# autowarefoundation/autoware_vision_pilot

Hardware: AMD Instinct MI355X
Metric: frames/sec (SceneSeg+Scene3D 1280x720, one camera per GPU: preprocess + shared encoder + 2 decoder(s) + decode per frame); p50 per-frame latency beside it (higher is better)
Workload: dtype fp16x3 (hi+lo fp16 pairs on the fp16 MFMA pipe, fp32 accumulate; fp32-class: floats within 1e-3 of the fp32 oracle, 0 class flips outside that float tolerance -- tie flips only, counted per pass in profiles/r06_parity_sweep.tsv); 1 GPU; BASELINE.json metric configuration: SceneSeg+Scene3D on one 1280x720 camera per GPU, batch 1, shared EfficientNet-B0 encoder (vp_create_shared), fp16x3; precision=fp16x3, parity_mode=True, frames_in_flight_per_gpu=3, net_input=1x3x320x640, gather=False

## Files before the change

autoware_vision_pilot_amd/csrc/engine_upconv.cpp:

```cpp
#include "engine_internal.hpp"

namespace vp {

namespace {

inline void tap_of(int q, int tt, int* a, int* d) {
  const int hr = q + tt - 1;
  const int o = hr >= 0 ? hr / 2 : -1;
  *d = hr - 2 * o;
  *a = o + 1 - q;
}

inline void split_half_d(double v, double pre, half_t* hi, half_t* lo, int keep_bits) {
  const double x = v * pre;
  if (!(std::fabs(x) <= 65504.0)) throw RangeError("composed up-sampling weight " + std::to_string(v) + " is outside the fp16 range the matrix pipe carries: re-scale the checkpoint");
  const half_t h = (half_t)x;
  *hi = h;
  *lo = truncate_lo((half_t)(x - (double)h), keep_bits);
}

}

void Engine::compose_upconv(const float* wt, const float* bt, const float* ws, const float* bs, const float* w3, const float* b3, int cin, int cm, int cout,
                            int cs, UpconvComposed* out) {
// ... 77 lines not shown
    std::vector<ComposeGemmParams> gv(gs.begin() + 9, gs.end());
    d_gv = dupload(gv);
    VP_HIP_CHECK(launch_compose_gemm(d_gv, 9, cout, 1, stream_));
  }
  out->wx.resize(n_wx);
  std::vector<double> wsb(n_ws), vs(cs > 0 ? (size_t)9 * cout : 0);
  copy_d2h(out->wx.data(), d_wx, n_wx * sizeof(double));
  copy_d2h(wsb.data(), d_ws, n_ws * sizeof(double));
  if (cs > 0) copy_d2h(vs.data(), d_vs, vs.size() * sizeof(double));
  for (void* q : {(void*)d_w3r, (void*)d_wtr, (void*)d_br, (void*)d_bsr, (void*)d_wx, (void*)d_ws, (void*)d_vs, (void*)d_gx, (void*)d_gs, (void*)d_gv})
    if (q) dfree(q);
  out->ws.assign((size_t)9 * cout * cs, 0.0);
  std::vector<double> V((size_t)9 * cout);
  for (int t = 0; t < 9; ++t)
    for (int co = 0; co < cout; ++co) {
      const double* row = wsb.data() + ((size_t)t * cout + co) * (cs + 1);
      for (int c = 0; c < cs; ++c) out->ws[((size_t)t * cout + co) * cs + c] = row[c];
      V[(size_t)t * cout + co] = row[cs] + (cs > 0 ? vs[(size_t)t * cout + co] : 0.0);
    }
  out->bias.assign((size_t)9 * cout, 0.0);
  for (int rc = 0; rc < 3; ++rc)
    for (int cc = 0; cc < 3; ++cc)
      for (int co = 0; co < cout; ++co) {
        double b = (double)b3[co];
        for (int ty = (rc == 0 ? 1 : 0); ty <= (rc == 2 ? 1 : 2); ++ty)
          for (int tx = (cc == 0 ? 1 : 0); tx <= (cc == 2 ? 1 : 2); ++tx) b += V[(size_t)(ty * 3 + tx) * cout + co];
        out->bias[(size_t)(rc * 3 + cc) * cout + co] = b;
      }
}

bool Engine::upconv_wanted() const { return !fp8_storage() && !dev_option_is("VP_UPCONV", '0') && (split() || !dev_option_is("VP_UPCONV_F16", '0')); }

Act* Engine::add_upconv(const std::string& name, const Act* in, const Act* skip_in, const std::vector<float>& wt, const std::vector<float>& bt,
                        const std::vector<float>& ws, const std::vector<float>& bs, const std::vector<float>& w3, const std::vector<float>& b3, int cm,
                        int cout, int act, int shape, int nsplit, const std::string& out_name) {
  const bool x1 = !split();
  if (x1 && in->C % 64 != 0) throw std::invalid_argument("composed up-sampling stage in an fp16 engine: input channels a multiple of 64: " + name);
  const int cin = in->Creal, cin_pad = in->C, cs = skip_in ? skip_in->Creal : 0, cs_pad = skip_in ? skip_in->C : 0;
  if (wt.size() != (size_t)cin * cm * 4 || bt.size() != (size_t)cm) throw std::runtime_error("convT weight size mismatch: " + name);
  if (w3.size() != (size_t)cout * cm * 9 || b3.size() != (size_t)cout) throw std::runtime_error("conv weight size mismatch: " + name);
  if (skip_in && (ws.size() != (size_t)cm * cs || bs.size() != (size_t)cm)) throw std::runtime_error("skip conv weight size mismatch: " + name);
  if (skip_in && (skip_in->H != in->H * 2 || skip_in->W != in->W * 2)) throw std::runtime_error("skip tensor size mismatch: " + name);
  for (const std::vector<float>* v : {&wt, &w3, skip_in ? &ws : nullptr})
    if (v)
      for (float x : *v)
        if (!(std::fabs(x) <= 65504.0f))
          throw RangeError("weight " + std::to_string(x) + " is outside the fp16 range the matrix pipe carries (|w| <= 65504): re-scale the checkpoint");
  UpconvComposed cw;
  compose_upconv(wt.data(), bt.data(), skip_in ? ws.data() : nullptr, skip_in ? bs.data() : nullptr, w3.data(), b3.data(), cin, cm, cout, cs, &cw);

  const int ncols = round_up(cout, 32), coutw = round_up(ncols, 128);
  const int cin_v = x1 ? cin_pad / 2 : cin_pad, cs_v = x1 ? round_up(cs_pad, 64) / 2 : cs_pad, chm = x1 ? 2 : 1, chunk_w = x1 ? 64 : 32;
  const int S = upconv_steps(cin_v, cs_v), n_chunks = upconv_chunks(cin_v, cs_v);
  std::vector<half_t> hi((size_t)4 * S * coutw * 32, (half_t)0.0f), lo(hi.size(), (half_t)0.0f);
  std::vector<float> post((size_t)4 * coutw, 1.0f), bias((size_t)9 * coutw, 0.0f);
  for (int k = 0; k < 9; ++k)
    for (int co = 0; co < cout; ++co) bias[(size_t)k * coutw + co] = (float)cw.bias[(size_t)k * cout + co];
  parallel_rows(4 * cout, [&](int r_begin, int r_end) {
    for (int r = r_begin; r < r_end; ++r) {
      const int phase = r / cout, co = r - phase * cout, py = phase >> 1, px = phase & 1;
      double amax = 0.0;
      for (int k = 0; k < 4; ++k) {
        const double* row = cw.wx.data() + ((size_t)(phase * 4 + k) * cout + co) * cin;
        for (int ci = 0; ci < cin; ++ci) amax = std::max(amax, std::fabs(row[ci]));
      }
      for (int t = 0; t < 9 && cs > 0; ++t) {
        const double* row = cw.ws.data() + ((size_t)t * cout + co) * cs;
        for (int c = 0; c < cs; ++c) amax = std::max(amax, std::fabs(row[c]));
      }
      const int sexp = prescale_exp((float)amax);
      const double pre = std::ldexp(1.0, sexp);
      post[(size_t)phase * coutw + co] = std::ldexp(1.0f, -sexp);
      for (int c = 0; c < n_chunks; ++c) {
        const UpconvChunk d = upconv_chunk(c, py, px, cin_v, cs_v);
        const int creal = d.skip ? cs : cin;
        for (int k = 0; k < d.nt; ++k) {
          const int a = d.a0 + (d.nb == 2 ? (k >> 1) : k), b = d.b0 + (d.nb == 2 ? (k & 1) : 0);
          const double* row;
          if (d.skip) {
            const int ty = d.qy != py ? 2 * a : 1, tx = d.qx != px ? 2 * b : 1;
            row = cw.ws.data() + ((size_t)(ty * 3 + tx) * cout + co) * cs;
          } else {
            row = cw.wx.data() + ((size_t)(phase * 4 + a * 2 + b) * cout + co) * cin;
          }
          for (int i = 0; i < chunk_w && chm * d.ch0 + i < creal; ++i) {
            const size_t dst = upconv_pack_index(phase, d.step0 + k, co, i & 31, S, coutw);
            if (x1) {
              half_t h, l;
              split_half_d(row[chm * d.ch0 + i], pre, &h, &l, wlo_keep_);
              (i >> 5 ? lo : hi)[dst] = h;
            } else {
              split_half_d(row[d.ch0 + i], pre, &hi[dst], &lo[dst], wlo_keep_);
            }
          }
        }
      }
    }
  });
  Act* out = new_act(out_name.empty() ? name : out_name, cout, in->H * 2, in->W * 2);
  UpconvParams p{};
  p.in_hi = in->hi;
  p.in_lo = x1 ? nullptr : in->lo;
  p.sk_hi = skip_in ? skip_in->hi : nullptr;
  p.sk_lo = (skip_in && !x1) ? skip_in->lo : nullptr;
  p.H = in->H;
  p.W = in->W;
  p.Cin = cin_pad;
  p.Cs = cs_pad;
  p.w_hi = dupload(hi);
  p.w_lo = dupload(lo);
  wbytes_[1] += 2 * (hi.size() + lo.size());
  p.bias = dupload(bias);
  p.wscale = dupload(post);
  p.CoutW = coutw;
  p.Ncols = ncols;
  p.Cstore = out->C;
  p.out_hi = out->hi;
  p.out_lo = x1 ? nullptr : out->lo;
  p.act = (x1 && act == ACT_GELU) ? ACT_GELU_F16 : act;
  const long long t16 = (long long)((in->H + 15) / 16) * ((in->W + 15) / 16), t8 = (long long)((in->H + 7) / 8) * ((in->W + 15) / 16);
  const int n_co = coutw / 128;
  int sh = shape;
  {
    int ot = -1, on = 0;
    if (sh < 0 && plan_override(name, &ot, &on)) {
      sh = ot;
      if (on > 0 && nsplit <= 0) nsplit = on;
    }
  }
  if (sh < 0) {
    const double eff6 = (double)in->H * in->W / (double)(t16 * 256), eff7 = (double)in->H * in->W / (double)(t8 * 128);
    const char* e = dev_option("VP_UPCONV_SHAPE");
    sh = e ? std::atoi(e) : ((eff7 > 1.1 * eff6 || cin_pad <= 128) ? 7 : 6);
  }
  if (sh != 6 && sh != 7) throw std::invalid_argument("composed up-sampling stage: shape 6 (16x16 patches, 8 waves) or 7 (8x16 patches, 4 waves): " + name);
  const long long blocks = (sh == 6 ? t16 : t8) * 4 * n_co;
  int ns = nsplit;
  if (ns <= 0) {
    const long long slots = sh == 6 ? 256 : 512;
    ns = (int)std::max<long long>(1, slots / blocks);
    const double slice_mb = 4.0 * in->H * in->W * coutw * 4.0 / 1e6;
    while (ns > 1 && ns * slice_mb > 26.0) --ns;
    while (ns > 1 && S / ns < 12) --ns;
    if (const char* e = dev_option("VP_UPCONV_NSPLIT")) ns = std::max(1, std::atoi(e));
  }
  ns = std::max(1, std::min(ns, n_chunks));
  p.nsplit = ns;
  {
    const long long px = sh == 6 ? 256 : 128, runs = ((long long)in->H * in->W + px - 1) / px;
    const char* e = dev_option("VP_UPCONV_COMPACT");
    const bool want = e ? e[0] == '1' : runs < (sh == 6 ? t16 : t8);
    p.compact = (!x1 && want && upconv_compact_fits(in->H, in->W, sh)) ? 1 : 0;
  }
  p.partial = ns > 1 ? static_cast<float*>(dalloc((size_t)ns * 4 * in->H * in->W * coutw * sizeof(float), false)) : nullptr;
  if (!upconv_supported(p, sh)) throw std::invalid_argument("composed up-sampling stage: shape not covered: " + name);
  Op op;
  op.name = name;
  op.kernel = std::string(x1 ? "upconv_x1" : "upconv_x3") + (sh == 6 ? "w8<co128,px256" : "w4<co128,px128") + (x1 ? ",k64>" : ">") + (ns > 1 ? "+splitk" : "");
  if (ns > 1) op.launch = "nsplit=" + std::to_string(ns);
  const double M2 = 4.0 * in->H * in->W;
  op.flops = 2.0 * (M2 * cin * cm + M2 * cs * cm + M2 * 9.0 * cm * cout);
  op.flops_executed = 2.0 * M2 * cout * (4.0 * cin + 9.0 * cs);
  op.bytes = (x1 ? 2.0 : 4.0) * ((M2 / 4 * cin + M2 * cs + M2 * cout) + cout * (16.0 * cin + 9.0 * cs));
  op.run = [p, sh](hipStream_t st) { return launch_upconv(p, sh, st); };
  op.writes = {out};
  ops_.push_back(std::move(op));
  return out;
}

}
```

autoware_vision_pilot_amd/csrc/kernels.hpp:

```cpp
#pragma once
#include "common.hpp"

namespace vp {

const char* dev_option(const char* key);
bool dev_option_is(const char* key, char first);

struct PreprocessParams {
  const uint8_t* frame;
  int stride;
  const int* xtab;
  const int* ytab;
  int out_h, out_w;
  int src_c[3];
  float mean[3], stdv[3];
  float* out;
  int norm_form;
};

struct PilResampleParams {
  const uint8_t* frame;
  int stride;
  int in_h, in_w, out_h, out_w;
  const int* hb;
// ... 239 lines not shown
  const float* w2;
  const float* b2;
  int sq, Creal;
  int frames;
};

struct MbBackParams {
  ActView in;
  SeParams se;
  const unsigned long long* zsums;
  const float* w2q;
  const float* b2;
  int sqp;
  const float* w;
  const float* bias;
  const float* wscale;
  ActView res;
  ActView out;
};

struct LetterboxParams {
  const uint8_t* frame;
  int stride;
  const int* xtab;
  const int* ytab;
  int new_w, new_h, pad_x, pad_y;
  int out_h, out_w;
  float* out;
};

struct Detection {
  float x1, y1, x2, y2, confidence;
  int class_id;
};

enum DetectRule { kDetectPerClass = 0, kDetectAgnostic = 1 };
struct DetectParams {
  const float* raw;
  int num_attrs, num_boxes;
  float conf_thresh, iou_thresh;
  float scale;
  int pad_x, pad_y, orig_w, orig_h;
  float* boxes;
  int* cls;
  Detection* out;
  int out_cap;
  int* count;
};
constexpr int kDetectMaxBoxes = 16384;

struct LetterboxPasteParams {
  const float* src;
  int new_w, new_h, pad_x, pad_y;
  int out_h, out_w;
  float* out;
};

struct FcParams {
  const float* x;
  const float* w;
  const uint8_t* w8;
  const float* wscale8;
  const float* b;
  float* out;
  int N, K, act;
  unsigned act_rows;
  int rows_kernel;
  const float* partial;
  int nslab, Kstride;
  float inv_hw;
};

bool fc_rows_ok(const FcParams& p);

struct CtxConv1Params {
  const float* map;
  int H, W;
  const float* w;
  const float* b;
  ActView out;
  int act;
  int scaled;
  float out_mul;
};

struct CtxExpConv1Params {
  FcParams fc;
  CtxConv1Params cv;
  int tile;
  int glanes;
};
bool ctx_exp_conv1_ok(const CtxExpConv1Params& p);
hipError_t launch_ctx_exp_conv1(const CtxExpConv1Params& p, hipStream_t st);

struct FusionParams {
  ActView f[5];
  int creal[5];
  int shift[5];
  ActView out;
  int Creal_out;
  int octets;
};
bool fusion_octets_ok(const FusionParams& p);

hipError_t launch_conv_gemm(const ConvGemmParams& p, int tile, int bk, bool split, hipStream_t st);
int conv_tile_co(int tile);
int conv_tile_px(int tile);
hipError_t launch_conv3x3_halo(const ConvGemmParams& p, int tile, bool split, hipStream_t st);
bool conv3x3_x3_supported(const ConvGemmParams& p, int shape);
hipError_t launch_conv3x3_x3(const ConvGemmParams& p, int shape, hipStream_t st);
int halo_tile_co(int tile);
int halo_tile_px(int tile);
int halo_tile_th(int tile);
bool conv3x3_f8_supported(const ConvGemmParams& p);
hipError_t launch_conv3x3_f8(const ConvGemmParams& p, hipStream_t st);
hipError_t launch_fp8_quantize(const half_t* in, size_t n, float mul, uint8_t* out, hipStream_t st);

int conv3x3_map_geometry(int H, int W);
bool conv3x3_map_shape_ok(int H, int W, int cin_pad, int coutw);
size_t conv3x3_map_pack_index(int co, int ci, int t, int cin_pad);
size_t conv3x3_map_pack_index_k32(int co, int ci, int t, int cin_pad);
bool conv3x3_map_supported(const ConvGemmParams& p);
hipError_t launch_conv3x3_map(const ConvGemmParams& p, hipStream_t st);
bool conv3x3_map2_shape_ok(int H, int W, int cin_pad, int coutw);
bool conv3x3_map2_supported(const ConvGemmParams& p);
size_t conv3x3_map2_pack_index(int co, int ci, int t, int cin_pad);
hipError_t launch_conv3x3_map2(const ConvGemmParams& p, hipStream_t st);
bool head_conv_supported(const ConvGemmParams& p);
hipError_t launch_head_conv(const ConvGemmParams& p, const void* zeros, hipStream_t st);
bool gemm_dma_shape_ok(int M, int ncols, int cin_pad, int cin2_pad, int cstore);
size_t gemm_dma_pack_index(int n, int k, int kw);
bool gemm_dma_supported(const ConvGemmParams& p, bool split);
hipError_t launch_gemm_dma(const ConvGemmParams& p, hipStream_t st);
bool convt_rs_supported(const ConvGemmParams& p, bool split);
int convt_rs_shape_case(int H, int W, int cin_pad, int cin2_pad, int ncols, int cstore);
hipError_t launch_convt_rs(const ConvGemmParams& p, hipStream_t st);
struct UpconvParams {
  const half_t* in_hi;
  const half_t* in_lo;
  const half_t* sk_hi;
  const half_t* sk_lo;
  int H, W, Cin, Cs;
  const half_t* w_hi;
  const half_t* w_lo;
  const float* bias;
  const float* wscale;
  int CoutW, Ncols, Cstore;
  half_t* out_hi;
  half_t* out_lo;
  int act;
  int nsplit;
  float* partial;
  int compact;
};
bool upconv_supported(const UpconvParams& p, int shape);
bool upconv_compact_fits(int H, int W, int shape);
struct UpconvChunk {
  int skip, ch0, qy, qx, nt, nb, a0, b0, step0;
};
__host__ __device__ inline UpconvChunk upconv_chunk(int c, int py, int px, int cin_pad, int cs_pad) {
  const int kcx = cin_pad >> 5, kcs = cs_pad >> 5;
  UpconvChunk d;
  if (c < kcx || kcs == 0) {
    d.skip = 0; d.ch0 = c << 5; d.qy = 0; d.qx = 0; d.nt = 4; d.nb = 2; d.a0 = 0; d.b0 = 0; d.step0 = 4 * c;
    return d;
  }
  const int r = c - kcx, cls = r / kcs, cc = r - cls * kcs;
  d.skip = 1;
  d.ch0 = cc << 5;
  d.qy = cls < 2 ? 1 - py : py;
  d.qx = (cls & 1) ? px : 1 - px;
  const int na = d.qy != py ? 2 : 1;
  d.nb = d.qx != px ? 2 : 1;
  d.a0 = na == 2 ? 0 : 1 - py;
  d.b0 = d.nb == 2 ? 0 : 1 - px;
  d.nt = na * d.nb;
  const int cls_step0 = cls == 0 ? 0 : (cls == 1 ? 4 : (cls == 2 ? 6 : 8));
  d.step0 = 4 * kcx + cls_step0 * kcs + cc * d.nt;
  return d;
}
__host__ __device__ inline int upconv_chunks(int cin_pad, int cs_pad) { return (cin_pad >> 5) + 4 * (cs_pad >> 5); }
__host__ __device__ inline int upconv_steps(int cin_pad, int cs_pad) { return 4 * (cin_pad >> 5) + 9 * (cs_pad >> 5); }
inline size_t upconv_pack_index(int phase, int step, int co, int i, int steps, int coutw) {
  const int i_sw = ((((i & 31) >> 3) ^ ((co >> 2) & 3)) << 3) | (i & 7);
  return (((size_t)phase * steps + step) * coutw + co) * 32 + i_sw;
}
hipError_t launch_upconv(const UpconvParams& p, int shape, hipStream_t st);
struct ComposeGemmParams {
  const float* a[4];
  const float* b[4];
  int pairs, M, N, K;
  double* c;
};
hipError_t launch_compose_gemm(const ComposeGemmParams* groups_dev, int n_groups, int M, int N, hipStream_t st);
hipError_t launch_preprocess(const PreprocessParams& p, hipStream_t st);
hipError_t launch_pil_resample(const PilResampleParams& p, hipStream_t st);
hipError_t launch_stem(const StemParams& p, hipStream_t st);
hipError_t launch_dwconv(const DwParams& p, hipStream_t st);
bool mbconv_front_supported(const MbFrontParams& p);
hipError_t launch_mbconv_front(const MbFrontParams& p, hipStream_t st);
hipError_t launch_letterbox(const LetterboxParams& p, hipStream_t st);
hipError_t launch_detect_nms(const DetectParams& p, DetectRule rule, hipStream_t st);
inline hipError_t launch_detect_decode_nms(const DetectParams& p, hipStream_t st) { return launch_detect_nms(p, kDetectPerClass, st); }
hipError_t launch_letterbox_paste(const LetterboxPasteParams& p, hipStream_t st);
bool mbconv_back_supported(const MbBackParams& p);
hipError_t launch_mbconv_back(const MbBackParams& p, hipStream_t st);
hipError_t launch_pool_partial(const PoolParams& p, hipStream_t st);
hipError_t launch_zero_u64(unsigned long long* p, size_t n, hipStream_t st);
constexpr int kSeMaxReplicas = 64;
hipError_t launch_se_gate_scale(const SeParams& se, const ScaleWParams& sw, hipStream_t st);
hipError_t launch_fc(const FcParams& p, hipStream_t st);
hipError_t launch_ctx_conv1(const CtxConv1Params& p, hipStream_t st);
hipError_t launch_fusion(const FusionParams& p, hipStream_t st);
hipError_t launch_decode_mask(const float* logits, int C, int HW, int mode, uint8_t* out, hipStream_t st);
hipError_t launch_resize_nearest(const uint8_t* src, int sw, const int* ytab, const int* xtab, int oh, int ow, uint8_t* dst,
                                 hipStream_t st);
hipError_t launch_resize_bilinear_f32(const float* src, int sw, const int* yi, const float* yf, const int* xi, const float* xf,
                                      int oh, int ow, float* dst, hipStream_t st);
hipError_t launch_minmax_f32(const float* src, size_t n, unsigned* mm, hipStream_t st);
constexpr int VP_PROBE_BLOCKS = 64;
hipError_t launch_finite_probe(const float* src, size_t n, unsigned* flags, hipStream_t st);
hipError_t launch_depth_colorize(const float* src, size_t n, const unsigned* mm, const uint8_t* lut, uint8_t* dst, hipStream_t st);
hipError_t launch_viz_blend(const uint8_t* mask, int mw, const int* ytab, const int* xtab, const uint8_t* frame, int stride, int oh, int ow,
                            const uint8_t* lut, int frame_is_rgb, uint8_t* dst, hipStream_t st);
hipError_t launch_nchw_to_act(const float* src, int Creal, const ActView& a, hipStream_t st);
hipError_t launch_act_to_nchw(const ActView& a, int Creal, float* dst, hipStream_t st, float mul = 1.0f);
hipError_t launch_act_absmax(const half_t* hi, const half_t* lo, int c, int h, int w, int c_pitch, unsigned* result, hipStream_t st);
constexpr int VP_HIST_BINS = 40, VP_HIST_EXP_MIN = -24, VP_HIST_WORDS = VP_HIST_BINS + 2;
hipError_t launch_act_exp_hist(const half_t* hi, const half_t* lo, int c, int h, int w, int c_pitch, unsigned long long* result, hipStream_t st);

hipError_t launch_chan_copy(const ActView& src, int src_off, const ActView& dst, int dst_off, int nch, hipStream_t st);
hipError_t launch_maxpool5(const ActView& src, int src_off, const ActView& dst, int dst_off, int nch, hipStream_t st);
bool sppf_pool_ok(const ActView& src, const ActView& dst, int nch);
hipError_t launch_sppf_pool(const ActView& src, const ActView& dst, int nch, hipStream_t st);
struct AttnParams {
  ActView qkv;
  ActView out;
  ActView vout;
  int heads, dk, dv;
  float scale;
  int qblock;
};
bool attention_block_ok(const AttnParams& p);
hipError_t launch_attention(const AttnParams& p, hipStream_t st);
struct DwPlainParams {
  ActView in, out;
  ActView add;
  const float* w;
  const float* b;
  int act;
  int scaled;
  float in_mul, add_mul, out_mul;
};
hipError_t launch_dwconv_plain(const DwPlainParams& p, hipStream_t st);

struct Upsample2CatParams {
  ActView a, b, out;
  int a_off, a_nch, b_off, b_nch;
};
bool upsample2_cat_ok(const Upsample2CatParams& p);
hipError_t launch_upsample2_cat(const Upsample2CatParams& p, hipStream_t st);
struct DetectHeadLevel {
  ActView box;
  ActView cls;
  int first;
  float stride;
  float box_mul, cls_mul;
};
struct DetectHeadParams {
  DetectHeadLevel lv[3];
  int nc, total;
  float* out;
  int scaled;
};
hipError_t launch_detect_head_decode(const DetectHeadParams& p, hipStream_t st);

struct RowpairConvParams {
  ActView in;
  int cin;
  const float* w;
  const float* b;
  ActView out;
  int replicate;
  int scaled;
  float in_mul, out_mul;
};
bool rowpair_conv_ok(const RowpairConvParams& p);
hipError_t launch_rowpair_conv(const RowpairConvParams& p, hipStream_t st);
struct LaneRowsHeadParams {
  ActView features;
  int cin;
  const float* w;
  const float* hw;
  float* out;
  int scaled;
  float in_mul;
};
bool lane_rows_head_ok(const LaneRowsHeadParams& p);
hipError_t launch_lane_rows_head(const LaneRowsHeadParams& p, hipStream_t st);

struct MetricRecord {
  int kind;
  unsigned I[3], P[3], G[3];
  unsigned nonfinite, n, kept;
  float q_lo, q_hi, q, mae, mel;
};
// ... 197 lines not shown
```

autoware_vision_pilot_amd/csrc/kernels_upconv.hip:

```cpp
#include <algorithm>
#include <cstdlib>

#include "conv_epilogue.hpp"
#include "lds_dma.hpp"

namespace vp {

namespace {

struct PixPhase {
  int y0, x0, H, W, py, px;
  __device__ __forceinline__ int operator()(int q) const {
    int rowbit, c;
    lane_to_px16(q & 31, rowbit, c);
    const int y = y0 + 2 * (q >> 5) + rowbit, x = x0 + c;
    return (y < H && x < W) ? (2 * y + py) * (2 * W) + 2 * x + px : -1;
  }
};
struct PixRun {
  int kA, kE, W, py, px;
  __device__ __forceinline__ int operator()(int q) const {
    int rowbit, c;
    lane_to_px16(q & 31, rowbit, c);
    const int k = kA + (q >> 5) * 32 + 16 * rowbit + c;
    if (k >= kE) return -1;
    const int y = k / W, x = k - y * W;
    return (2 * y + py) * (2 * W) + 2 * x + px;
  }
};
constexpr int upconv_halo_bytes(int TH, bool CPT) { return (CPT && TH == 8) ? 192 * 80 : (TH + 2) * 18 * 80; }
constexpr int upconv_halo_capacity(int nth) { return 3 * nth / 4; }
__device__ __forceinline__ int bias_class(int m, int H2, int W2) {
  const int Y = m / W2, X = m - Y * W2;
  return (Y == 0 ? 0 : (Y == H2 - 1 ? 2 : 1)) * 3 + (X == 0 ? 0 : (X == W2 - 1 ? 2 : 1));
}

}

#define VP_WAIT_VMCNT_RT(N)                       \
  do {                                            \
    const int n_ = (N);                           \
    if (n_ >= 16) { VP_WAIT_VMCNT(16); }          \
    else if (n_ >= 14) { VP_WAIT_VMCNT(14); }     \
    else if (n_ >= 12) { VP_WAIT_VMCNT(12); }     \
    else if (n_ >= 10) { VP_WAIT_VMCNT(10); }     \
    else if (n_ >= 8) { VP_WAIT_VMCNT(8); }       \
    else if (n_ >= 6) { VP_WAIT_VMCNT(6); }       \
    else if (n_ >= 4) { VP_WAIT_VMCNT(4); }       \
    else if (n_ >= 2) { VP_WAIT_VMCNT(2); }       \
    else { VP_WAIT_VMCNT(0); }                    \
  } while (0)

template <int CO_TILE, int TH, int WCO, int WPX, bool HDB, int ACT, bool SPLITK, bool X1 = false, int ABL = 0, bool CPT = false>
__global__ __launch_bounds__(64 * WCO * WPX, 2) void upconv_x3_kernel(const UpconvParams p) {
  constexpr int NTH = 64 * WCO * WPX;
  constexpr int TW = 16, ROWB = 80, HWD = TW + 2, HPX = (TH + 2) * HWD, PX = TH * TW;
  constexpr int HALO_BYTES = upconv_halo_bytes(TH, CPT), WROW = 64, W_BYTES = CO_TILE * WROW;
  constexpr int HCHUNKS = HPX * 4, HP = (HCHUNKS + NTH - 1) / NTH;
  constexpr int MT = CO_TILE / WCO / 32, NT = PX / WPX / 32;
  constexpr int NHB = HDB ? 2 : 1;
  constexpr int PL = 2;
  constexpr int HSTRIDE = HALO_BYTES;
  static_assert(MT >= 1 && NT >= 1 && HP <= 3, "tile shape");
  extern __shared__ __attribute__((aligned(16))) char smem[];
  char* const halo_base = smem;
  char* const w_base = smem + NHB * PL * HSTRIDE;

  const int tid = threadIdx.x, lane = tid & 63, wave = tid >> 6;
  const int wco = wave / WPX, wpx = wave % WPX;
  const int tiles_x = (p.W + TW - 1) / TW;
  const int n_px_tiles = CPT ? (p.H * p.W + PX - 1) / PX : tiles_x * ((p.H + TH - 1) / TH);
  const int n_co_tiles = p.CoutW / CO_TILE;
  int vid;
  {
    const int nwg = gridDim.x, q = nwg >> 3, r = nwg & 7, xcd = blockIdx.x & 7;
    vid = (xcd < r ? xcd * (q + 1) : r * (q + 1) + (xcd - r) * q) + (blockIdx.x >> 3);
  }
  int tile_px, tile_co, phase, zsplit = 0;
  if constexpr (SPLITK) {
    tile_px = vid % n_px_tiles;
    int rest = vid / n_px_tiles;
    tile_co = rest % n_co_tiles;
    rest /= n_co_tiles;
    phase = rest & 3;
    zsplit = rest >> 2;
  } else {
    tile_co = vid % n_co_tiles;
    const int rest = vid / n_co_tiles;
    phase = rest & 3;
    tile_px = rest >> 2;
  }
  const int py = phase >> 1, px = phase & 1;
  const int tyi = tile_px / tiles_x, txi = tile_px - tyi * tiles_x;
  const int y0 = tyi * TH, x0 = txi * TW;
  const int kA = tile_px * PX, kE = min(kA + PX, p.H * p.W);
  const int yA = kA / p.W, xA = kA - yA * p.W, yE = (kE - 1) / p.W, xE = (kE - 1) - yE * p.W;
  const int hrp = CPT ? p.W * ROWB + 256 : HWD * ROWB;
  const int tpy = CPT ? 0 : py, tpx = CPT ? 0 : px;
  const int co0 = tile_co * CO_TILE;
  const int CinV = X1 ? p.Cin >> 1 : p.Cin, CsV = X1 ? ((p.Cs + 63) >> 6) << 5 : p.Cs;
  constexpr int CHM = X1 ? 2 : 1;
  const half_t* const in_p1 = X1 ? p.in_hi + 32 : p.in_lo;
  const half_t* const sk_p1 = X1 ? p.sk_hi + 32 : p.sk_lo;
#define VP_SK_DEAD1(D) (X1 && (D).skip && CHM * (D).ch0 + 32 >= p.Cs)
  const int n_chunks = upconv_chunks(CinV, CsV);
  int cA = 0, cB = n_chunks;
  if constexpr (SPLITK) {
    cA = (int)(((long long)n_chunks * zsplit) / p.nsplit);
    cB = (int)(((long long)n_chunks * (zsplit + 1)) / p.nsplit);
  }

  const int h_lds0 = (tid >> 2) * ROWB + (tid & 3) * 16;
  constexpr int NW = NTH / 64, WPIECES = W_BYTES / 1024 / NW;
  static_assert(W_BYTES % (1024 * NW) == 0, "weight tile splits into 1 KiB pieces per wave");
  const size_t w_step = (size_t)p.CoutW * 32;
  typedef unsigned int u32x4 __attribute__((ext_vector_type(4)));
  const u32x4 zero4 = {0u, 0u, 0u, 0u};
  int b_ofs0;
  int b_ofs[NT];
  int nlj = NT;
  {
    int rowbit, c;
    lane_to_px16(lane & 31, rowbit, c);
    b_ofs0 = ((2 * (wpx * NT) + rowbit) * HWD + c) * ROWB + (lane >> 5) * 16;
    if constexpr (CPT) {
#pragma unroll
      for (int j = 0; j < NT; ++j) {
        int k = kA + (wpx * NT + j) * 32 + 16 * rowbit + c;
        if (k >= kE) k = kA;
        const int y = k / p.W, x = k - y * p.W;
        b_ofs[j] = (y - yA) * hrp + (x - xA) * ROWB + (lane >> 5) * 16;
      }
      nlj = __builtin_amdgcn_readfirstlane(min(NT, max(0, (kE - kA + 31) / 32 - wpx * NT)));
    }
  }
  const int a_swz = ((lane & 31) >> 2) & 3;
  const int a_ofs0 = (wco * 32 + (lane & 31)) * WROW + (((lane >> 5) ^ a_swz) << 4);

  int h_gx[HP], h_gs[HP], h_ls[HP];
#pragma unroll
  for (int pc = 0; pc < HP; ++pc) {
    const int hidx = tid + NTH * pc;
    const int hp = hidx >> 2, ch = hidx & 3;
    int gy, gx;
    bool ok;
    if constexpr (CPT) {
      const int gw = p.W + 2, lg = py * gw + xA + px + hp, cnt = (yE - yA + 1) * gw + xE - xA + 2;
      const int r = lg / gw, cc = lg - r * gw;
      gy = yA - 1 + r;
      gx = cc - 1;
      ok = hp < cnt && (unsigned)gy < (unsigned)p.H && (unsigned)gx < (unsigned)p.W;
      h_ls[pc] = hp < cnt ? (r - py) * hrp + (cc - xA - px) * ROWB + ch * 16 : -1;
    } else {
      const int hy = hp / HWD, hx = hp - hy * HWD;
      gy = y0 - 1 + hy;
      gx = x0 - 1 + hx;
      ok = hidx < HCHUNKS && (unsigned)gy < (unsigned)p.H && (unsigned)gx < (unsigned)p.W && hy >= py && hy <= py + TH && hx >= px && hx <= px + TW;
    }
    h_gx[pc] = ok ? (gy * p.W + gx) * p.Cin + ch * 8 : -1;
    h_gs[pc] = ok ? (4 * gy * p.W + 2 * gx) * p.Cs + ch * 8 : -1;
  }
  const UpconvChunk dA = upconv_chunk(cA, py, px, CinV, CsV);
  const int S = (cB < n_chunks ? upconv_chunk(cB, py, px, CinV, CsV).step0 : upconv_steps(CinV, CsV)) - dA.step0;
  const size_t w_goff0 = ((size_t)phase * upconv_steps(CinV, CsV) + dA.step0) * w_step + co0 * 32 + wave * 512 + lane * 8;

  f32x16_t acc[MT][NT];
#pragma unroll
  for (int i = 0; i < MT; ++i)
#pragma unroll
    for (int j = 0; j < NT; ++j)
#pragma unroll
      for (int r = 0; r < 16; ++r) acc[i][j][r] = 0.0f;

  h8_t fa[2][MT], fal[2][MT], fb[2][NT], fbl[2][NT];
  u32x4 rh_hi[HP], rh_lo[HP];
#pragma unroll
  for (int r = 0; r < HP; ++r) rh_hi[r] = rh_lo[r] = zero4;

#define VP_DMA_W(WOFS, SIDX)                                                                 \
  if (!(ABL & 128) || (SIDX) < 2) {                                                          \
    const size_t base_ = (size_t)(SIDX) * w_step + w_goff0;                                  \
    char* dst_ = w_base + (WOFS) + wave * 1024;                                              \
    _Pragma("unroll") for (int pc = 0; pc < WPIECES; ++pc) {                                 \
      VP_GLOBAL_LOAD_LDS16(p.w_hi + base_ + pc * NW * 512, dst_ + pc * NW * 1024);           \
      VP_GLOBAL_LOAD_LDS16(p.w_lo + base_ + pc * NW * 512, dst_ + W_BYTES + pc * NW * 1024); \
    }                                                                                        \
  }
#define VP_LOAD_H(D)                                                                         \
  if (!(ABL & 1) || abl_prologue) {                                                          \
    const half_t* sh_ = (D).skip ? p.sk_hi : p.in_hi;                                        \
    const half_t* sl_ = (D).skip ? (VP_SK_DEAD1(D) ? p.sk_hi : sk_p1) : in_p1;               \
    const int add_ = (D).skip ? ((D).qy * 2 * p.W + (D).qx) * p.Cs + CHM * (D).ch0 : CHM * (D).ch0; \
    _Pragma("unroll") for (int pc = 0; pc < HP; ++pc) {                                      \
      const int g_ = (D).skip ? h_gs[pc] : h_gx[pc];                                         \
      const int o_ = (g_ >= 0 ? g_ + add_ : 0);                                              \
      rh_hi[pc] = *reinterpret_cast<const u32x4*>(sh_ + o_);                                 \
      rh_lo[pc] = *reinterpret_cast<const u32x4*>(sl_ + o_);                                 \
    }                                                                                        \
  }
#define VP_STORE_H(BUF, DEAD1)                                                               \
  if (!(ABL & 1) || abl_prologue)                                                            \
  _Pragma("unroll") for (int pc = 0; pc < HP; ++pc) {                                        \
    if (CPT ? h_ls[pc] >= 0 : tid + NTH * pc < HCHUNKS) {                                    \
      char* dst_ = halo_base + (BUF) * PL * HSTRIDE + (CPT ? h_ls[pc] : h_lds0 + pc * (NTH / 4) * ROWB); \
      *reinterpret_cast<u32x4*>(dst_) = h_gx[pc] >= 0 ? rh_hi[pc] : zero4;                   \
      *reinterpret_cast<u32x4*>(dst_ + HSTRIDE) = (h_gx[pc] >= 0 && !(DEAD1)) ? rh_lo[pc] : zero4; \
    }                                                                                        \
  }
#define VP_READ_FRAGS(SET, WPTR, HPTR, TAPOFS)                                               \
  {                                                                                          \
    const char* wsrc_ = (WPTR) + (a_ofs0 ^ ((SET) * 32));                                    \
    if (!CPT || nlj > 0)                                                                     \
    _Pragma("unroll") for (int i = 0; i < MT; ++i) {                                         \
      fa[SET][i] = *reinterpret_cast<const h8_t*>(wsrc_ + i * WCO * 32 * WROW);              \
      fal[SET][i] = *reinterpret_cast<const h8_t*>(wsrc_ + W_BYTES + i * WCO * 32 * WROW);   \
    }                                                                                        \
    if constexpr (CPT) {                                                                     \
      const char* hsrc_ = (HPTR) + (TAPOFS) + (SET) * 32;                                    \
      _Pragma("unroll") for (int j = 0; j < NT; ++j) {                                       \
        if (j >= nlj) continue;                                                              \
        fb[SET][j] = *reinterpret_cast<const h8_t*>(hsrc_ + b_ofs[j]);                       \
        fbl[SET][j] = *reinterpret_cast<const h8_t*>(hsrc_ + HSTRIDE + b_ofs[j]);            \
      }                                                                                      \
    } else {                                                                                 \
      const char* hsrc_ = (HPTR) + b_ofs0 + (TAPOFS) + (SET) * 32;                           \
      _Pragma("unroll") for (int j = 0; j < NT; ++j) {                                       \
        fb[SET][j] = *reinterpret_cast<const h8_t*>(hsrc_ + j * 2 * HWD * ROWB);             \
        fbl[SET][j] = *reinterpret_cast<const h8_t*>(hsrc_ + HSTRIDE + j * 2 * HWD * ROWB);  \
      }                                                                                      \
    }                                                                                        \
  }
#define VP_MFMA_RANGE(SET, Q0, Q1)                                                           \
  _Pragma("unroll") for (int q_ = (Q0); q_ < (Q1); ++q_) {                                   \
    const int i = q_ / NT, j = q_ % NT;                                                      \
    if constexpr (CPT) { if (j >= nlj) continue; }        \
    if constexpr ((ABL & 2) != 0) { acc[i][j][0] += (float)fa[SET][i][0] + (float)fal[SET][i][1] + (float)fb[SET][j][2] + (float)fbl[SET][j][3]; continue; } \
    if constexpr (X1) {                      \
      acc[i][j] = __builtin_amdgcn_mfma_f32_32x32x16_f16(fa[SET][i], fb[SET][j], acc[i][j], 0, 0, 0);   \
      acc[i][j] = __builtin_amdgcn_mfma_f32_32x32x16_f16(fal[SET][i], fbl[SET][j], acc[i][j], 0, 0, 0); \
      continue;                                                                              \
    }                                                                                        \
    acc[i][j] = __builtin_amdgcn_mfma_f32_32x32x16_f16(fal[SET][i], fb[SET][j], acc[i][j], 0, 0, 0); \
    acc[i][j] = __builtin_amdgcn_mfma_f32_32x32x16_f16(fa[SET][i], fbl[SET][j], acc[i][j], 0, 0, 0); \
    acc[i][j] = __builtin_amdgcn_mfma_f32_32x32x16_f16(fa[SET][i], fb[SET][j], acc[i][j], 0, 0, 0);  \
  }
#define VP_TAP_OFS(D, K) ((tpy + (D).a0 + ((D).nb == 2 ? ((K) >> 1) : (K))) * hrp + (tpx + (D).b0 + ((D).nb == 2 ? ((K) & 1) : 0)) * ROWB)

  bool abl_prologue = true;
  VP_LOAD_H(dA)
  VP_STORE_H(0, VP_SK_DEAD1(dA))
  VP_DMA_W(0, 0)
  if (S > 1) VP_DMA_W(PL * W_BYTES, 1)
  VP_WAIT_VMCNT(0);
  __syncthreads();
  UpconvChunk d = dA;
  UpconvChunk dn = dA;
  if (cA + 1 < cB) {
    dn = upconv_chunk(cA + 1, py, px, CinV, CsV);
    VP_LOAD_H(dn)
  }
  VP_READ_FRAGS(0, w_base, halo_base, VP_TAP_OFS(d, 0))
  abl_prologue = false;

  int c = cA, t = 0, s = 0, hb = 0;
  int w_cur = 0, w_nxt = PL * W_BYTES, w_fre = 2 * PL * W_BYTES;
#define VP_STEP(KIND, PREVLD)                                                                \
  {                                                                                          \
    const int tap_cur_ = VP_TAP_OFS(d, t);                                                   \
    const int tap_nxt_ = (KIND) == 0 ? VP_TAP_OFS(d, t + 1) : ((KIND) == 3 ? tap_cur_ : VP_TAP_OFS(dn, 0)); \
    const char* hbuf = halo_base + (HDB ? hb : 0) * PL * HSTRIDE;                            \
    const char* hbuf_next = (HDB && (KIND) != 0) ? halo_base + (hb ^ 1) * PL * HSTRIDE : hbuf; \
     \
     \
     \
    if constexpr (HDB && ((KIND) == 1 || (KIND) == 2)) { VP_STORE_H(hb ^ 1, VP_SK_DEAD1(dn)) }   \
     \
    if (s + 2 < S) VP_DMA_W(w_fre, s + 2)                                                    \
    __builtin_amdgcn_sched_barrier(0);                                                       \
    VP_MFMA_RANGE(0, 0, MT * NT / 2)                                                         \
    __builtin_amdgcn_sched_barrier(0);                                                       \
    VP_READ_FRAGS(1, w_base + w_cur, hbuf, tap_cur_)                                         \
    __builtin_amdgcn_sched_barrier(0);   \
    UpconvChunk dnn = dn;                                                                    \
    if constexpr (HDB && (KIND) == 1) {                                                      \
      dnn = upconv_chunk(c + 2, py, px, CinV, CsV);                                        \
      VP_LOAD_H(dnn)                                                                         \
    }                                                                                        \
    VP_MFMA_RANGE(0, MT * NT / 2, MT * NT)                                                   \
    __builtin_amdgcn_sched_barrier(0);                                                       \
     \
     \
    {                                                                                        \
      const int dma_n = s + 2 < S ? PL * WPIECES : 0;                                        \
      const int ld_prev = ((PREVLD) && t == 0) ? PL * HP : 0;                                \
      const int ld_this = (HDB && (KIND) == 1) ? PL * HP : 0;                                \
      VP_WAIT_VMCNT_RT(dma_n + ld_prev + ld_this);                                           \
    }                                                                                        \
     \
    VP_LDS_BARRIER();                                                                        \
    if constexpr (!HDB && ((KIND) == 1 || (KIND) == 2)) {                                    \
       \
       \
      VP_STORE_H(0, VP_SK_DEAD1(dn))                                                         \
      VP_LDS_BARRIER();                                                                      \
      if constexpr ((KIND) == 1) {                                                           \
        dnn = upconv_chunk(c + 2, py, px, CinV, CsV);                                      \
        VP_LOAD_H(dnn)                                                                       \
      }                                                                                      \
    }                                                                                        \
           \
    VP_READ_FRAGS(0, w_base + w_nxt, hbuf_next, tap_nxt_)                                    \
    __builtin_amdgcn_sched_barrier(0);                                                       \
    VP_MFMA_RANGE(1, 0, MT * NT)                                                             \
    __builtin_amdgcn_sched_barrier(0);                                                       \
                                    \
    {                                                                                        \
      const int w_old = w_cur;                                                               \
      w_cur = w_nxt;                                                                         \
      w_nxt = w_fre;                                                                         \
      w_fre = w_old;                                                                         \
    }                                                                                        \
    ++s;                                                                                     \
    if constexpr ((KIND) == 0) {                                                             \
      ++t;                                                                                   \
    } else {                                                                                 \
      ++c;                                                                                   \
      t = 0;                                                                                 \
      d = dn;                                                                                \
      dn = dnn;                                                                              \
      hb ^= 1;                                                                               \
    }                                                                                        \
  }
  while (c + 2 < cB) {
    while (t + 1 < d.nt) VP_STEP(0, true)
    VP_STEP(1, true)
  }
  if (c + 1 < cB) {
    while (t + 1 < d.nt) VP_STEP(0, true)
    VP_STEP(2, true)
  }
  while (t + 1 < d.nt) VP_STEP(0, false)
  VP_STEP(3, false)
#undef VP_STEP
#undef VP_SK_DEAD1
#undef VP_TAP_OFS
#undef VP_MFMA_RANGE
#undef VP_READ_FRAGS
#undef VP_STORE_H
#undef VP_LOAD_H
#undef VP_DMA_W

  const auto pix = [&] {
    if constexpr (CPT) return PixRun{kA, kE, p.W, py, px};
    else return PixPhase{y0, x0, p.H, p.W, py, px};
  }();
  if constexpr ((ABL & 16) != 0) {
    if (p.H == -12345) {
#pragma unroll
      for (int i = 0; i < MT; ++i)
#pragma unroll
        for (int j = 0; j < NT; ++j)
#pragma unroll
          for (int r = 0; r < 16; ++r) p.partial[(i * NT + j) * 16 + r + tid * 64] = acc[i][j][r];
    }
    return;
  }
  if constexpr (SPLITK) {
    const int M2 = 4 * p.H * p.W;
#pragma unroll
    for (int j = 0; j < NT; ++j) {
      const int m = pix((wpx * NT + j) * 32 + (lane & 31));
      if (m < 0) continue;
      float* row = p.partial + ((size_t)zsplit * M2 + m) * p.CoutW + co0 + 4 * (lane >> 5);
#pragma unroll
      for (int i = 0; i < MT; ++i)
#pragma unroll
        for (int g = 0; g < 4; ++g) {
          const f32x4_t v = {acc[i][j][4 * g + 0], acc[i][j][4 * g + 1], acc[i][j][4 * g + 2], acc[i][j][4 * g + 3]};
          *reinterpret_cast<f32x4_t*>(row + (i * WCO + wco) * 32 + 8 * g) = v;
        }
    }
    return;
  } else {
    constexpr int PITCH = CO_TILE * 2 + 16, STAGE_PLANE = PX * PITCH;
    static_assert(PL * STAGE_PLANE <= NHB * PL * HSTRIDE + 3 * PL * W_BYTES, "stage fits the main buffers");
    const float* const wsc = p.wscale + (size_t)phase * p.CoutW + co0;
    f32x4_t bb[NT][MT][4], sc[MT][4];
    int qpix[NT];
#pragma unroll
    for (int j = 0; j < NT; ++j) {
      qpix[j] = (wpx * NT + j) * 32 + (lane & 31);
      const int m = pix(qpix[j]);
      const float* const bsrc = p.bias + (size_t)(m >= 0 ? bias_class(m, 2 * p.H, 2 * p.W) : 4) * p.CoutW + co0;
#pragma unroll
      for (int i = 0; i < MT; ++i)
#pragma unroll
        for (int g = 0; g < 4; ++g) bb[j][i][g] = *reinterpret_cast<const f32x4_t*>(bsrc + (i * WCO + wco) * 32 + 4 * (lane >> 5) + 8 * g);
    }
#pragma unroll
    for (int i = 0; i < MT; ++i)
#pragma unroll
      for (int g = 0; g < 4; ++g) sc[i][g] = *reinterpret_cast<const f32x4_t*>(wsc + (i * WCO + wco) * 32 + 4 * (lane >> 5) + 8 * g);
    __syncthreads();
#pragma unroll
    for (int j = 0; j < NT; ++j) {
#pragma unroll
      for (int i = 0; i < MT; ++i) {
        const int cl = (i * WCO + wco) * 32 + 4 * (lane >> 5);
        char* row = smem + qpix[j] * PITCH + cl * 2;
#pragma unroll
        for (int g = 0; g < 4; ++g) {
          h4_t h, l;
#pragma unroll
          for (int r = 0; r < 4; ++r) {
            const float x = apply_act(fmaf(acc[i][j][4 * g + r], sc[i][g][r], bb[j][i][g][r]), ACT);
            h[r] = (half_t)x;
            if constexpr (!X1) l[r] = (half_t)(x - (float)h[r]);
          }
          *reinterpret_cast<h4_t*>(row + g * 16) = h;
          if constexpr (!X1) *reinterpret_cast<h4_t*>(row + STAGE_PLANE + g * 16) = l;
        }
      }
    }
    __syncthreads();
    constexpr int CPR = CO_TILE / 8, RPI = NTH / CPR;
    static_assert(NTH % CPR == 0 && PX % RPI == 0, "row loop shape");
    const int c8 = tid % CPR, r0 = tid / CPR;
    const int co = co0 + c8 * 8;
    if (co >= p.Ncols) return;
#pragma unroll 4
    for (int r = r0; r < PX; r += RPI) {
      const int m = pix(r);
      if (m < 0) continue;
      if constexpr ((ABL & 32) != 0) { if (p.H != -12345) continue; }
      const size_t o = (size_t)m * p.Cstore + co;
      *reinterpret_cast<h8_t*>(p.out_hi + o) = *reinterpret_cast<const h8_t*>(smem + r * PITCH + c8 * 16);
      if constexpr (!X1) *reinterpret_cast<h8_t*>(p.out_lo + o) = *reinterpret_cast<const h8_t*>(smem + STAGE_PLANE + r * PITCH + c8 * 16);
    }
  }
}

__global__ __launch_bounds__(256) void upconv_finish_kernel(const UpconvParams p) {
  const int H2 = 2 * p.H, W2 = 2 * p.W, M2 = H2 * W2;
  const int groups = p.Ncols >> 3;
  const long long t = (long long)blockIdx.x * 256 + threadIdx.x;
  if (t >= (long long)M2 * groups) return;
  const int m = (int)(t / groups), co = (int)(t % groups) * 8;
  float v[8] = {0.f, 0.f, 0.f, 0.f, 0.f, 0.f, 0.f, 0.f};
  for (int z = 0; z < p.nsplit; ++z) {
    const float* src = p.partial + ((size_t)z * M2 + m) * p.CoutW + co;
    const f32x4_t q0 = *reinterpret_cast<const f32x4_t*>(src), q1 = *reinterpret_cast<const f32x4_t*>(src + 4);
#pragma unroll
    for (int r = 0; r < 4; ++r) {
      v[r] += q0[r];
      v[4 + r] += q1[r];
    }
  }
  const int Y = m / W2, X = m - Y * W2;
  const int phase = (Y & 1) * 2 + (X & 1);
  const float* b = p.bias + (size_t)bias_class(m, H2, W2) * p.CoutW + co;
  const float* s = p.wscale + (size_t)phase * p.CoutW + co;
  h8_t hi, lo;
#pragma unroll
  for (int r = 0; r < 8; ++r) {
    const float x = apply_act(fmaf(v[r], s[r], b[r]), p.act);
    hi[r] = (half_t)x;
    lo[r] = (half_t)(x - (float)hi[r]);
  }
  const size_t o = (size_t)m * p.Cstore + co;
  *reinterpret_cast<h8_t*>(p.out_hi + o) = hi;
  if (p.out_lo) *reinterpret_cast<h8_t*>(p.out_lo + o) = lo;
}

bool upconv_compact_fits(int H, int W, int shape) {
  if ((shape != 6 && shape != 7) || H < 1 || W < 1 || (long long)H * W >= (1 << 24)) return false;
  const int PX = shape == 6 ? 256 : 128, nth = shape == 6 ? 512 : 256, th = shape == 6 ? 16 : 8;
  for (int kA = 0; kA < H * W; kA += PX) {
    const int kE = std::min(kA + PX, H * W), yA = kA / W, xA = kA - yA * W, yE = (kE - 1) / W, xE = (kE - 1) - yE * W;
    const long long cnt = (long long)(yE - yA + 1) * (W + 2) + xE - xA + 2;
    const long long bytes = (long long)(yE - yA + 1) * (W * 80 + 256) + (xE - xA + 1) * 80 + 80;
    if (cnt > upconv_halo_capacity(nth) || bytes > upconv_halo_bytes(th, true)) return false;
  }
  return true;
}

bool upconv_supported(const UpconvParams& p, int shape) {
  if (shape != 6 && shape != 7) return false;
  if (p.compact && (p.in_lo == nullptr || !upconv_compact_fits(p.H, p.W, shape))) return false;
  const bool x1 = p.in_lo == nullptr;
  if (!(p.in_hi && p.w_hi && p.w_lo && p.bias && p.wscale && p.out_hi && (x1 ? p.out_lo == nullptr : p.out_lo != nullptr))) return false;
  if (p.H < 1 || p.W < 1 || p.Cin < (x1 ? 64 : 32) || p.Cin % (x1 ? 64 : 32) != 0 || p.Cs % 32 != 0 || p.Cs < 0) return false;
  if (p.Cs > 0 && !(p.sk_hi && (x1 ? p.sk_lo == nullptr : p.sk_lo != nullptr))) return false;
  if (p.CoutW % 128 != 0 || p.Ncols % 8 != 0 || p.Ncols > p.CoutW || p.Cstore < p.Ncols) return false;
  if (!(p.act == (x1 ? ACT_GELU_F16 : ACT_GELU) || p.act == ACT_NONE)) return false;
  if (p.nsplit < 1 || p.nsplit > (x1 ? upconv_chunks(p.Cin >> 1, ((p.Cs + 63) >> 6) << 5) : upconv_chunks(p.Cin, p.Cs))) return false;
// ... 96 lines not shown
```

autoware_vision_pilot_amd/csrc/options.cpp:

```cpp
#include <atomic>
#include <cstring>
#include <deque>
#include <map>
#include <mutex>
#include <string>

#include "../../include/vp_hip.h"
#include "kernels.hpp"

namespace vp {
namespace {
std::mutex g_mu;
std::atomic<int> g_count{0};
std::map<std::string, const char*> g_opts;
std::deque<std::string> g_arena;
bool g_version_stale = true;
std::deque<std::string> g_versions;

const char* const kKeys[] = {"VP_MBCONV_FUSE", "VP_MBCONV_BACK", "VP_PROJ_SPLIT", "VP_FUSE_DECODE", "VP_AUTOTUNE", "VP_HEAD_CONV", "VP_CONVT_RS",
                             "VP_CONV3X3", "VP_HEAD_TILE5", "VP_X3_TILE", "VP_X3_MIN_WGS", "VP_MAP3X3", "VP_NSPLIT_PCT", "VP_NSPLIT_FORCE", "VP_X3_C64",
                             "VP_GEMM_DMA", "VP_GEMM_DMA_NSPLIT", "VP_CONVT_TILE", "VP_CONVT_BK", "VP_FUSE_SKIP", "VP_CONVT_RS_GROUPS", "VP_F16_BIG",
                             "VP_CTX3", "VP_MAP_TAPSPLIT", "VP_ATTN_BLOCK", "VP_F16_MAP", "VP_MAP_NSPLIT_PCT", "VP_MAP2", "VP_MAP2_SLOTS", "VP_X3_T16", "VP_MAP2_CAP_MB", "VP_MAP2_MIN_REGIONS", "VP_CTX_FUSE", "VP_MAP_MAX_M", "VP_F16_MIN_WGS", "VP_CONVT_RS_GROUPS_K288", "VP_PLAN_TARGET", "VP_UPCONV", "VP_UPCONV_SHAPE", "VP_UPCONV_NSPLIT", "VP_PLAN_OVERRIDE", "VP_WLO_KEEP_BITS", "VP_UPCONV_F16", "VP_UPCONV_COMPACT"};
}

const char* dev_option(const char* key) {
  if (g_count.load(std::memory_order_acquire) == 0) return nullptr;
  std::lock_guard<std::mutex> lk(g_mu);
  auto it = g_opts.find(key);
  return it == g_opts.end() ? nullptr : it->second;
}
bool dev_option_is(const char* key, char first) {
  const char* v = dev_option(key);
  return v != nullptr && v[0] == first;
}

}

extern "C" {

int vp_set_option(const char* key, const char* value) {
  if (!key) return VP_ERR_ARG;
  bool known = false;
  for (const char* k : vp::kKeys) known = known || std::strcmp(k, key) == 0;
  if (!known) return VP_ERR_ARG;
  if (value && std::strcmp(key, "VP_PLAN_TARGET") == 0 && std::strcmp(value, "latency") != 0 && std::strcmp(value, "throughput") != 0) return VP_ERR_ARG;
  std::lock_guard<std::mutex> lk(vp::g_mu);
  if (!value) {
    vp::g_opts.erase(key);
  } else {
    vp::g_arena.emplace_back(value);
    vp::g_opts[key] = vp::g_arena.back().c_str();
  }
  vp::g_version_stale = true;
  vp::g_count.store((int)vp::g_opts.size(), std::memory_order_release);
  return VP_OK;
}

const char* vp_get_option(const char* key) { return key ? vp::dev_option(key) : nullptr; }

void vp_clear_options(void) {
  std::lock_guard<std::mutex> lk(vp::g_mu);
  vp::g_opts.clear();
  vp::g_version_stale = true;
  vp::g_count.store(0, std::memory_order_release);
}

const char* vp_version(void) {
  std::lock_guard<std::mutex> lk(vp::g_mu);
  if (vp::g_version_stale) {
    std::string s = "libvp_hip 0.5 (gfx950; options:";
    if (vp::g_opts.empty()) s += " none";
    for (const auto& kv : vp::g_opts) s += std::string(" ") + kv.first + "=" + kv.second;
    s += ")";
    if (vp::g_versions.empty() || vp::g_versions.back() != s) vp::g_versions.push_back(s);
    vp::g_version_stale = false;
  }
  return vp::g_versions.back().c_str();
}

}
```

Baseline: 561.0 frames/s.

## Add statically unrolled tap schedule for up-conv input-channel chunks

Adds a specialised main loop for the composed up-sampling kernel that unrolls the four taps of each input-channel chunk with compile-time step kinds. This lets vmcnt waits use immediate counts instead of a runtime ladder, and interleaves weight DMA, halo loads and MFMA halves at fixed positions. The wave index used for LDS DMA addressing is also made wave-uniform through readfirstlane. The path is on by default for non-x1 kernels and can be disabled with an option. It adds code size and register pressure, and the hand-computed wait counts risk a correctness or hazard error if they are miscounted.

```diff
diff --git a/autoware_vision_pilot_amd/csrc/engine_upconv.cpp b/autoware_vision_pilot_amd/csrc/engine_upconv.cpp
--- a/autoware_vision_pilot_amd/csrc/engine_upconv.cpp
+++ b/autoware_vision_pilot_amd/csrc/engine_upconv.cpp
@@ -253,6 +253,7 @@
     const bool want = e ? e[0] == '1' : runs < (sh == 6 ? t16 : t8);
     p.compact = (!x1 && want && upconv_compact_fits(in->H, in->W, sh)) ? 1 : 0;
   }
+  p.xstatic = dev_option_is("VP_UPCONV_STATIC", '0') ? 0 : 1;
   p.partial = ns > 1 ? static_cast<float*>(dalloc((size_t)ns * 4 * in->H * in->W * coutw * sizeof(float), false)) : nullptr;
   if (!upconv_supported(p, sh)) throw std::invalid_argument("composed up-sampling stage: shape not covered: " + name);
   Op op;
diff --git a/autoware_vision_pilot_amd/csrc/kernels.hpp b/autoware_vision_pilot_amd/csrc/kernels.hpp
--- a/autoware_vision_pilot_amd/csrc/kernels.hpp
+++ b/autoware_vision_pilot_amd/csrc/kernels.hpp
@@ -415,6 +415,7 @@
   int nsplit;
   float* partial;
   int compact;
+  int xstatic;
 };
 bool upconv_supported(const UpconvParams& p, int shape);
 bool upconv_compact_fits(int H, int W, int shape);
diff --git a/autoware_vision_pilot_amd/csrc/kernels_upconv.hip b/autoware_vision_pilot_amd/csrc/kernels_upconv.hip
--- a/autoware_vision_pilot_amd/csrc/kernels_upconv.hip
+++ b/autoware_vision_pilot_amd/csrc/kernels_upconv.hip
@@ -50,6 +50,8 @@
     else if (n_ >= 2) { VP_WAIT_VMCNT(2); }       \
     else { VP_WAIT_VMCNT(0); }                    \
   } while (0)
+
+constexpr int upconv_vmcnt_imm(int n) { return n >= 16 ? 16 : (n & ~1); }
 
 template <int CO_TILE, int TH, int WCO, int WPX, bool HDB, int ACT, bool SPLITK, bool X1 = false, int ABL = 0, bool CPT = false>
 __global__ __launch_bounds__(64 * WCO * WPX, 2) void upconv_x3_kernel(const UpconvParams p) {
@@ -177,10 +179,11 @@
 #pragma unroll
   for (int r = 0; r < HP; ++r) rh_hi[r] = rh_lo[r] = zero4;
 
+  const int wave_u = __builtin_amdgcn_readfirstlane(wave);
 #define VP_DMA_W(WOFS, SIDX)                                                                 \
   if (!(ABL & 128) || (SIDX) < 2) {                                                          \
     const size_t base_ = (size_t)(SIDX) * w_step + w_goff0;                                  \
-    char* dst_ = w_base + (WOFS) + wave * 1024;                                              \
+    char* dst_ = w_base + (WOFS) + wave_u * 1024;                                            \
     _Pragma("unroll") for (int pc = 0; pc < WPIECES; ++pc) {                                 \
       VP_GLOBAL_LOAD_LDS16(p.w_hi + base_ + pc * NW * 512, dst_ + pc * NW * 1024);           \
       VP_GLOBAL_LOAD_LDS16(p.w_lo + base_ + pc * NW * 512, dst_ + W_BYTES + pc * NW * 1024); \
@@ -331,16 +334,101 @@
       hb ^= 1;                                                                               \
     }                                                                                        \
   }
-  while (c + 2 < cB) {
-    while (t + 1 < d.nt) VP_STEP(0, true)
-    VP_STEP(1, true)
-  }
-  if (c + 1 < cB) {
-    while (t + 1 < d.nt) VP_STEP(0, true)
-    VP_STEP(2, true)
-  }
-  while (t + 1 < d.nt) VP_STEP(0, false)
-  VP_STEP(3, false)
+#define VP_XTAP(T) (CPT ? ((T) >> 1) * hrp + ((T) & 1) * ROWB : (((T) >> 1) * HWD + ((T) & 1)) * ROWB)
+#define VP_XSTEP(T, KIND, DMA, LDPREV)                                                       \
+  {                                                                                          \
+    const char* hbuf = halo_base + (HDB ? hb : 0) * PL * HSTRIDE + ph_ofs;                   \
+    const char* hbuf_next = hbuf;                                                            \
+    int tap_nxt_ = (KIND) == 0 ? VP_XTAP((T) + 1) : VP_XTAP(T);                              \
+    if constexpr ((KIND) == 1 || (KIND) == 2) {                                              \
+      hbuf_next = halo_base + (HDB ? (hb ^ 1) : 0) * PL * HSTRIDE;                           \
+      tap_nxt_ = VP_TAP_OFS(dn, 0);                                                          \
+    }                                                                                        \
+    if constexpr (HDB && ((KIND) == 1 || (KIND) == 2)) { VP_STORE_H(hb ^ 1, VP_SK_DEAD1(dn)) }   \
+    if constexpr ((DMA) == 1) { VP_DMA_W(w_fre, s + 2) }                                     \
+    if constexpr ((DMA) == 2) { if (s + 2 < S) VP_DMA_W(w_fre, s + 2) }                      \
+    __builtin_amdgcn_sched_barrier(0);                                                       \
+    VP_MFMA_RANGE(0, 0, MT * NT / 2)                                                         \
+    __builtin_amdgcn_sched_barrier(0);                                                       \
+    VP_READ_FRAGS(1, w_base + w_cur, hbuf, VP_XTAP(T))                                       \
+    __builtin_amdgcn_sched_barrier(0);                                                       \
+    UpconvChunk dnn = dn;                                                                    \
+    if constexpr ((KIND) == 1) {                                                             \
+      if (c + 2 < kcx) dnn.ch0 = (c + 2) << 5;                      \
+      else dnn = c + 2 == kcx ? dS0 : dS1;                                                   \
+    }                                                                                        \
+    if constexpr (HDB && (KIND) == 1) { VP_LOAD_H(dnn) }                                     \
+    VP_MFMA_RANGE(0, MT * NT / 2, MT * NT)                                                   \
+    __builtin_amdgcn_sched_barrier(0);                                                       \
+    {                                                                                        \
+      constexpr int nw_ = ((DMA) == 1 ? PL * WPIECES : 0) + ((LDPREV) ? PL * HP : 0) + ((HDB && (KIND) == 1) ? PL * HP : 0); \
+      if constexpr ((DMA) == 2) {                                                            \
+        if (s + 2 < S) { VP_WAIT_VMCNT(upconv_vmcnt_imm(nw_ + PL * WPIECES)); }              \
+        else { VP_WAIT_VMCNT(upconv_vmcnt_imm(nw_)); }                                       \
+      } else {                                                                               \
+        VP_WAIT_VMCNT(upconv_vmcnt_imm(nw_));                                                \
+      }                                                                                      \
+    }                                                                                        \
+    VP_LDS_BARRIER();                                                                        \
+    if constexpr (!HDB && ((KIND) == 1 || (KIND) == 2)) {                                    \
+      VP_STORE_H(0, VP_SK_DEAD1(dn))                                                         \
+      VP_LDS_BARRIER();                                                                      \
+      if constexpr ((KIND) == 1) { VP_LOAD_H(dnn) }                                          \
+    }                                                                                        \
+    VP_READ_FRAGS(0, w_base + w_nxt, hbuf_next, tap_nxt_)                                    \
+    __builtin_amdgcn_sched_barrier(0);                                                       \
+    VP_MFMA_RANGE(1, 0, MT * NT)                                                             \
+    __builtin_amdgcn_sched_barrier(0);                                                       \
+    {                                                                                        \
+      const int w_old = w_cur;                                                               \
+      w_cur = w_nxt;                                                                         \
+      w_nxt = w_fre;                                                                         \
+      w_fre = w_old;                                                                         \
+    }                                                                                        \
+    ++s;                                                                                     \
+    if constexpr ((KIND) != 0) {                                                             \
+      ++c;                                                                                   \
+      d = dn;                                                                                \
+      dn = dnn;                                                                              \
+      hb ^= 1;                                                                               \
+    }                                                                                        \
+  }
+  bool done = false;
+  if constexpr (!X1) {
+    const int kcx = CinV >> 5;
+    if (p.xstatic && cA < kcx) {
+      const int ph_ofs = tpy * hrp + tpx * ROWB;
+      UpconvChunk dS0 = dA, dS1 = dA;
+      if (kcx < cB) {
+        dS0 = upconv_chunk(kcx, py, px, CinV, CsV);
+        dS1 = upconv_chunk(kcx + 1, py, px, CinV, CsV);
+      }
+      while (c + 2 < cB && c < kcx) {
+        VP_XSTEP(0, 0, 1, true) VP_XSTEP(1, 0, 1, false) VP_XSTEP(2, 0, 1, false) VP_XSTEP(3, 1, 1, false)
+      }
+      if (c + 2 == cB && c < kcx) {
+        VP_XSTEP(0, 0, 1, true) VP_XSTEP(1, 0, 1, false) VP_XSTEP(2, 0, 1, false) VP_XSTEP(3, 2, 2, false)
+      }
+      if (c + 1 == cB && c < kcx) {
+        VP_XSTEP(0, 0, 1, false) VP_XSTEP(1, 0, 1, false) VP_XSTEP(2, 0, 0, false) VP_XSTEP(3, 3, 0, false)
+        done = true;
+      }
+    }
+  }
+#undef VP_XSTEP
+#undef VP_XTAP
+  if (!done) {
+    while (c + 2 < cB) {
+      while (t + 1 < d.nt) VP_STEP(0, true)
+      VP_STEP(1, true)
+    }
+    if (c + 1 < cB) {
+      while (t + 1 < d.nt) VP_STEP(0, true)
+      VP_STEP(2, true)
+    }
+    while (t + 1 < d.nt) VP_STEP(0, false)
+    VP_STEP(3, false)
+  }
 #undef VP_STEP
 #undef VP_SK_DEAD1
 #undef VP_TAP_OFS
diff --git a/autoware_vision_pilot_amd/csrc/options.cpp b/autoware_vision_pilot_amd/csrc/options.cpp
--- a/autoware_vision_pilot_amd/csrc/options.cpp
+++ b/autoware_vision_pilot_amd/csrc/options.cpp
@@ -20,7 +20,7 @@
 const char* const kKeys[] = {"VP_MBCONV_FUSE", "VP_MBCONV_BACK", "VP_PROJ_SPLIT", "VP_FUSE_DECODE", "VP_AUTOTUNE", "VP_HEAD_CONV", "VP_CONVT_RS",
                              "VP_CONV3X3", "VP_HEAD_TILE5", "VP_X3_TILE", "VP_X3_MIN_WGS", "VP_MAP3X3", "VP_NSPLIT_PCT", "VP_NSPLIT_FORCE", "VP_X3_C64",
                              "VP_GEMM_DMA", "VP_GEMM_DMA_NSPLIT", "VP_CONVT_TILE", "VP_CONVT_BK", "VP_FUSE_SKIP", "VP_CONVT_RS_GROUPS", "VP_F16_BIG",
-                             "VP_CTX3", "VP_MAP_TAPSPLIT", "VP_ATTN_BLOCK", "VP_F16_MAP", "VP_MAP_NSPLIT_PCT", "VP_MAP2", "VP_MAP2_SLOTS", "VP_X3_T16", "VP_MAP2_CAP_MB", "VP_MAP2_MIN_REGIONS", "VP_CTX_FUSE", "VP_MAP_MAX_M", "VP_F16_MIN_WGS", "VP_CONVT_RS_GROUPS_K288", "VP_PLAN_TARGET", "VP_UPCONV", "VP_UPCONV_SHAPE", "VP_UPCONV_NSPLIT", "VP_PLAN_OVERRIDE", "VP_WLO_KEEP_BITS", "VP_UPCONV_F16", "VP_UPCONV_COMPACT"};
+                             "VP_CTX3", "VP_MAP_TAPSPLIT", "VP_ATTN_BLOCK", "VP_F16_MAP", "VP_MAP_NSPLIT_PCT", "VP_MAP2", "VP_MAP2_SLOTS", "VP_X3_T16", "VP_MAP2_CAP_MB", "VP_MAP2_MIN_REGIONS", "VP_CTX_FUSE", "VP_MAP_MAX_M", "VP_F16_MIN_WGS", "VP_CONVT_RS_GROUPS_K288", "VP_PLAN_TARGET", "VP_UPCONV", "VP_UPCONV_SHAPE", "VP_UPCONV_NSPLIT", "VP_PLAN_OVERRIDE", "VP_WLO_KEEP_BITS", "VP_UPCONV_F16", "VP_UPCONV_COMPACT", "VP_UPCONV_STATIC"};
 }
 
 const char* dev_option(const char* key) {
```

After: 566.2 frames/s (median of 6 runs). About the same (+0.9%).
